# ParBLiSS/kmerind

Measured on AMD Instinct MI355X. Metric: kmers_per_sec_indexed, higher is better.
Workload: dtype u64

## Files before the change

### kmerind_amd/csrc/kmi_superkmer.h

```cpp
#pragma once

namespace kmi {

constexpr int kRecNShift = 38, kRecHashShift = 43;
constexpr uint64_t kSkPadW1 = ~0ull;
constexpr int kRecEdgeShift = 32;
constexpr uint32_t kSkEdgeWindows = 3;
__device__ __forceinline__ uint32_t rec_hash18(uint64_t w1) { return (uint32_t)(w1 >> kRecHashShift) & 0x3ffffu; }
__device__ __forceinline__ uint32_t rec_fine_sub(uint64_t w1) { return (rec_hash18(w1) >> 3) & 127u; }

constexpr int kSkThreads = 512;
constexpr int kSkRoundTiles = 24;
constexpr int kSkListCap = 32;

struct SkRound {
  uint64_t t; uint32_t ei, total; uint32_t eo[kSkRoundTiles + 1]; uint64_t nt; uint32_t nei;
};
__device__ __forceinline__ bool sk_plan(const uint32_t *__restrict__ ent_cnt, uint64_t te, uint64_t t, uint32_t ei, SkRound &r) {
  while (t < te && ei >= ent_cnt[t]) { ++t; ei = 0; }
  if (t >= te) return false;
  r.t = t; r.ei = ei; r.eo[0] = 0;
  r.nt = t + kSkRoundTiles; r.nei = 0;
  bool cut = false;
#pragma unroll
// ... 406 lines not shown
constexpr int kSlackLCap = kSlackLT + (kSlackLineRecs - 1) * kSubPerCoarse;
__global__ __launch_bounds__(kPartThreads) void sk_scatter_fine_slack_lines_kernel(const uint64_t *__restrict__ recs, uint64_t *__restrict__ out,
                                                                                 const uint64_t *__restrict__ wg_off, const uint64_t *__restrict__ coarse_end,
                                                                                 uint32_t groups, const uint64_t *__restrict__ fine_region,
                                                                                 const uint32_t *__restrict__ fine_cap, uint32_t *__restrict__ fine_cnt,
                                                                                 uint32_t *__restrict__ fine_kmers, uint32_t *__restrict__ flags) {
  constexpr int NB = kSubPerCoarse, T = kSlackLT, PT = T / kPartThreads, SCAP = kSlackLCap, L = kSlackLineRecs, MAXG = SCAP / L + NB;
  static_assert(kPartThreads / NB == L && T % kPartThreads == 0, "one carry slot per thread: eight threads per bucket");
  __shared__ ulonglong2 s_stage[SCAP];
  __shared__ uint32_t s_cnt[NB];
  __shared__ uint32_t s_k[NB];
  __shared__ uint32_t s_lofs[NB];
  __shared__ uint32_t s_emit[NB];
  __shared__ uint32_t s_old[NB];
  __shared__ uint32_t s_lbase[NB];
  __shared__ uint64_t s_dst[NB];
  __shared__ uint32_t s_part[NB / kWave];
  __shared__ uint32_t s_ng;
  __shared__ uint8_t s_linebkt[MAXG];
  const uint32_t gpp = groups / kFineParts;
  const uint32_t c = blockIdx.x / kFineParts, h = blockIdx.x % kFineParts;
  const uint64_t b = wg_off[(uint64_t)(h * gpp) * kNumCoarse + c];
  const uint64_t e = (h + 1 < (uint32_t)kFineParts) ? wg_off[(uint64_t)((h + 1) * gpp) * kNumCoarse + c] : coarse_end[c];
  if (b >= e) return;
  const uint64_t region = fine_region[c];
  const uint32_t cap = fine_cap[c];
  if (threadIdx.x < NB) { s_cnt[threadIdx.x] = 0; s_k[threadIdx.x] = 0; }
  const uint32_t cb = threadIdx.x / L, cj = threadIdx.x % L;
  ulonglong2 carry = make_ulonglong2(0, 0);
  uint32_t my_carry = 0;
  lds_barrier();
  const ulonglong2 *src = reinterpret_cast<const ulonglong2 *>(recs);
  ulonglong2 raw[PT];
  auto load_tile = [&](uint64_t t0) {
#pragma unroll
    for (int j = 0; j < PT; ++j) {
      uint64_t i = t0 + (uint64_t)j * kPartThreads + threadIdx.x;
      i = (i < e) ? i : e - 1;
      raw[j] = src[i];
    }
  };
  auto take = [&](uint32_t f, uint32_t n) -> uint64_t {
    const uint32_t at = atomicAdd(&fine_cnt[c * NB + f], n);
    if ((uint64_t)at + n > (uint64_t)cap) { atomicOr(&flags[34], 1u); return ~0ull; }
    return region + (uint64_t)f * cap + at;
  };
  load_tile(b);
  for (uint64_t t0 = b; t0 < e; t0 += T) {
    const uint32_t nt = (uint32_t)((e - t0 < (uint64_t)T) ? (e - t0) : (uint64_t)T);
    ulonglong2 rec[PT];
    uint32_t bk[PT], rk[PT];
#pragma unroll
    for (int j = 0; j < PT; ++j) {
      const uint32_t li = j * kPartThreads + threadIdx.x;
      rec[j] = raw[j];
      bk[j] = 0xffffffffu;
      if (li < nt) {
        bk[j] = rec_fine_sub(rec[j].y);
        rk[j] = atomicAdd(&s_cnt[bk[j]], 1u);
        atomicAdd(&s_k[bk[j]], ((uint32_t)(rec[j].y >> kRecNShift) & 31u) + 1u);
      }
    }
    if (t0 + T < e) load_tile(t0 + T);
    lds_barrier();
    uint32_t cnt = 0, emit = 0, ng = 0, inc = 0;
    if (threadIdx.x < NB) {
      cnt = s_cnt[threadIdx.x];
      const uint32_t km = s_k[threadIdx.x];
      s_k[threadIdx.x] = 0;
      emit = cnt & ~(uint32_t)(L - 1);
      ng = emit / L;
      inc = wave_inclusive_sum_dpp(cnt | (ng << 16));
      if (lane_id() == kWave - 1) s_part[wave_id()] = inc;
      if (km) atomicAdd(&fine_kmers[c * NB + threadIdx.x], km);
      s_dst[threadIdx.x] = emit ? take(threadIdx.x, emit) : ~0ull;
    }
    lds_barrier();
    if (threadIdx.x < NB) {
      const uint32_t pre = wave_id() ? s_part[0] : 0u;
      const uint32_t ex = pre + inc - (cnt | (ng << 16));
      const uint32_t lo = ex & 0xffffu, lb = ex >> 16;
      s_lofs[threadIdx.x] = lo; s_emit[threadIdx.x] = emit; s_old[threadIdx.x] = my_carry; s_lbase[threadIdx.x] = lb;
      for (uint32_t i = 0; i < ng; ++i) s_linebkt[lb + i] = (uint8_t)threadIdx.x;
      if (threadIdx.x == NB - 1) s_ng = lb + ng;
      s_cnt[threadIdx.x] = cnt - emit;
      my_carry = cnt - emit;
    }
    lds_barrier();
    if (cj < s_old[cb]) s_stage[s_lofs[cb] + cj] = carry;
#pragma unroll
    for (int j = 0; j < PT; ++j)
      if (bk[j] != 0xffffffffu) s_stage[s_lofs[bk[j]] + rk[j]] = rec[j];
    lds_barrier();
    {
      const uint32_t n_groups = s_ng, l8 = threadIdx.x & (uint32_t)(L - 1);
      for (uint32_t g = threadIdx.x / L; g < n_groups; g += kPartThreads / L) {
        const uint32_t f = s_linebkt[g];
        const uint64_t d = s_dst[f];
        const uint32_t i = (g - s_lbase[f]) * L + l8;
        if (d != ~0ull) reinterpret_cast<ulonglong2 *>(out)[d + i] = s_stage[s_lofs[f] + i];
      }
      const uint32_t rem = s_cnt[cb], base = s_lofs[cb] + s_emit[cb];
      if (cj < rem) carry = s_stage[base + cj];
    }
    lds_barrier();
  }
  {
    if (threadIdx.x < NB) s_dst[threadIdx.x] = my_carry ? take(threadIdx.x, (uint32_t)L) : ~0ull;
    lds_barrier();
    const uint32_t rem = s_cnt[cb];
    const uint64_t d = s_dst[cb];
    if (rem && d != ~0ull) reinterpret_cast<ulonglong2 *>(out)[d + cj] = cj < rem ? carry : make_ulonglong2(kEmptyKey, kSkPadW1);
  }
}

__global__ __launch_bounds__(1024) void sk_zero_kernel(uint32_t *__restrict__ a, uint32_t na, uint32_t *__restrict__ b, uint32_t nb,
                                                     uint32_t *__restrict__ c, uint32_t nc, uint32_t *__restrict__ flags, uint32_t f0, uint32_t f1,
                                                     uint32_t g0, uint32_t g1) {
  const uint32_t i = blockIdx.x * blockDim.x + threadIdx.x, stride = gridDim.x * blockDim.x;
  for (uint32_t x = i; x < na; x += stride) a[x] = 0;
  for (uint32_t x = i; x < nb; x += stride) b[x] = 0;
  for (uint32_t x = i; x < nc; x += stride) c[x] = 0;
  if (i >= f0 && i < f1) flags[i] = 0;
  if (i >= g0 && i < g1) flags[i] = 0;
}

__global__ __launch_bounds__(kPartThreads) void sk_recv_hist_kernel(const uint64_t *__restrict__ recs, uint64_t n, uint32_t *__restrict__ wg_hist,
                                                                   unsigned long long *__restrict__ n_kmers) {
  __shared__ uint32_t s_h[kNumCoarse];
  __shared__ unsigned long long s_k;
  if (threadIdx.x < kNumCoarse) s_h[threadIdx.x] = 0;
  if (threadIdx.x == 0) s_k = 0ull;
  lds_barrier();
  const uint64_t chunk = part_chunk(n, gridDim.x, PartCfg<2>::TILE);
  const uint64_t b = (uint64_t)blockIdx.x * chunk, e = (b + chunk < n) ? b + chunk : n;
  unsigned long long km = 0;
  for (uint64_t i = b + threadIdx.x; i < e; i += blockDim.x) {
    const uint64_t w1 = recs[2 * i + 1];
    atomicAdd(&s_h[rec_hash18(w1) >> 10], 1u);
    km += ((uint32_t)(w1 >> kRecNShift) & 31u) + 1u;
  }
  km = wave_reduce_sum(km);
  if (lane_id() == 0 && km) atomicAdd(&s_k, km);
  lds_barrier();
  if (threadIdx.x < kNumCoarse) wg_hist[(uint64_t)blockIdx.x * kNumCoarse + threadIdx.x] = s_h[threadIdx.x];
  if (threadIdx.x == 0 && s_k) atomicAdd(n_kmers, s_k);
}

#ifndef KMI_SK_H1
#define KMI_SK_H1 1536
#endif
#ifndef KMI_SK_T1_DUP
#define KMI_SK_T1_DUP 0.5f
#endif
#ifndef KMI_SK_FILL
#define KMI_SK_FILL 80
#endif
#ifndef KMI_SK_NT
#define KMI_SK_NT 1024
#endif
#ifndef KMI_SK_LDS_KB
#define KMI_SK_LDS_KB 160
#endif
#ifndef KMI_SK_HASH24
#define KMI_SK_HASH24 1
#endif
__device__ __forceinline__ uint32_t sk_slot_hash(uint64_t key) {
#if KMI_SK_HASH24
  const uint32_t lo = (uint32_t)key, hi = (uint32_t)(key >> 32);
  uint32_t h = __umul24(lo, 0x9E3779u);
  h += __umul24(__builtin_amdgcn_alignbit(hi, lo, 24), 0x85EBCBu);
  h += __umul24(hi >> 16, 0xC2B2AFu);
#else
  uint32_t h = ((uint32_t)key ^ ((uint32_t)(key >> 32) * 0x85EBCA6Bu)) * 0x9E3779B1u;
#endif
  h ^= h >> 15;
  return h;
}
__device__ __forceinline__ uint32_t sk_slot_of(uint32_t h, uint32_t cap) { return __umul24(h >> 16, cap) >> 16; }

#ifndef KMI_SK_PROBE_ATTR
#define KMI_SK_PROBE_ATTR __forceinline__
#endif
__device__ KMI_SK_PROBE_ATTR uint32_t sk_probe_insert(lds_u64_t *tkeys, lds_u32_t *tvals, lds_u32_t *distinct, lds_u32_t *overflow,
                                                         const lds_u64_t *q, const lds_u32_t *qw, uint32_t first, uint32_t cnt,
                                                         uint32_t cap, uint32_t last, uint32_t limit, uint32_t pending) {
  const uint32_t lane = lane_id();
  bool claimed = false;
  if (lane < cnt) {
    const uint64_t key = q[first + lane];
    const uint32_t wt = qw[first + lane];
    const uint32_t s0 = sk_slot_of(sk_slot_hash(key), cap);
    uint32_t s = s0;
    uint64_t c = __atomic_load_n(&tkeys[s], __ATOMIC_RELAXED);
    for (;;) {
      while (c != key && c != kEmptyKey && s - s0 < 64u) { ++s; c = __atomic_load_n(&tkeys[s], __ATOMIC_RELAXED); }
      if (c == key) break;
      if (c != kEmptyKey || s >= last) { *overflow = 1; s = last; break; }
      uint64_t expected = kEmptyKey;
      if (__atomic_compare_exchange_n(&tkeys[s], &expected, key, false, __ATOMIC_RELAXED, __ATOMIC_RELAXED)) { claimed = true; break; }
      c = expected;
    }
    __atomic_fetch_add(&tvals[s], wt, __ATOMIC_RELAXED);
  }
  const unsigned long long cm = __ballot(claimed);
  const uint32_t add = (uint32_t)__popcll(cm) + pending;
  if (add >= 16u || (add && cnt < 64u)) {
    if (lane == 0 && __atomic_fetch_add(distinct, add, __ATOMIC_RELAXED) + add >= limit) *overflow = 1;
    return 0u;
  }
  return add;
}


#ifndef KMI_SK_OVF
#define KMI_SK_OVF 448
#endif
constexpr int kSkOvf = KMI_SK_OVF;
#ifndef KMI_SK_TICKET_PLAIN
#define KMI_SK_TICKET_PLAIN 1
#endif
#ifndef KMI_SK_EMIT_BLOCK
#define KMI_SK_EMIT_BLOCK 1
#endif
template <int OWN_>
struct SkTab2 {
  static constexpr int NT = KMI_SK_NT, NWAVES = NT / kWave;
  static constexpr int OWN = OWN_;
  static constexpr int H1 = KMI_SK_H1, S1 = H1 + 64, L1 = H1 * 3 / 4;
  static constexpr int FIXED = NWAVES * (OWN + kMissQ * 12) + S1 * 20 + kSkOvf * 16 + 2560;
  static constexpr int S2 = ((KMI_SK_LDS_KB * 1024 - FIXED) / 12) / 64 * 64;
  static constexpr int CAP2 = S2 - 64, LIMIT2 = CAP2 * KMI_SK_FILL / 100;
};

template <bool CANON, int OWN_, bool SPECIAL>
#ifndef KMI_SK_MIN_WAVES
#define KMI_SK_MIN_WAVES 4
#endif
__global__ __launch_bounds__(KMI_SK_NT, KMI_SK_MIN_WAVES) void sk_reduce_kernel(const uint64_t *__restrict__ recs, const uint64_t *__restrict__ rec_off, uint32_t k,
                                                        const uint64_t *__restrict__ kmer_off ,
                                                        uint64_t *__restrict__ tmp_keys, uint32_t *__restrict__ tmp_vals,
                                                        uint32_t *__restrict__ out_cnt, uint32_t *__restrict__ flags,
                                                        uint32_t *__restrict__ queue , uint32_t n_buckets,
                                                        uint32_t start_bits, uint32_t lp, float inv_dup,
                                                        const uint64_t *__restrict__ fine_region = nullptr, const uint32_t *__restrict__ fine_cap = nullptr,
                                                        const uint32_t *__restrict__ fine_cnt = nullptr) {
  auto records_of = [&](uint32_t bb, uint64_t &lo, uint64_t &hi) {
    if (fine_cnt) {
      const uint32_t cap = fine_cap[bb >> 7], cnt = fine_cnt[bb];
      lo = fine_region[bb >> 7] + (uint64_t)(bb & 127u) * cap; hi = lo + (cnt < cap ? cnt : cap);
    }
    else { lo = rec_off[bb]; hi = rec_off[bb + 1]; }
  };
  using T = SkTab2<OWN_>;
  constexpr int NWAVES = T::NWAVES;
  constexpr uint64_t W1_INIT = ~0ull;
  enum { C_DIST = 0, C_OVF = 1, C_SPC = 2, C_SPS = 3, C_EMIT = 4, C_SP = 5, C_OVN = 6, C_T1N = 8, C_LVL = 9, C_NEXT = 10  };
  __shared__ uint64_t s_tk[T::S2];
  __shared__ uint32_t s_tv[T::S2];
  __shared__ ulonglong2 s_r[T::S1];
  __shared__ uint32_t s_rc[T::S1];
  __shared__ ulonglong2 s_ovf[kSkOvf];
  __shared__ uint64_t s_missq[NWAVES * kMissQ];
  __shared__ uint32_t s_missw[NWAVES * kMissQ];
  __shared__ uint8_t s_own[NWAVES * T::OWN];
  __shared__ uint32_t s_ctl[12];
  __shared__ uint32_t s_stack[320];
  const uint32_t lane = lane_id(), wv = wave_id();
  lds_u64_t *const tkeys = (lds_u64_t *)s_tk;
  lds_u32_t *const tvals = (lds_u32_t *)s_tv;
  lds_u32_t *const tdist = (lds_u32_t *)&s_ctl[C_DIST];
  lds_u32_t *const tovf = (lds_u32_t *)&s_ctl[C_OVF];
  uint64_t *const mq = s_missq + wv * kMissQ;
  uint32_t *const mw = s_missw + wv * kMissQ;
  uint8_t *const wown = s_own + wv * T::OWN;
  const uint32_t kb = 2u * k;
  const uint32_t kmask_hi = kb >= 64u ? 0xffffffffu : ((1u << (kb - 32u)) - 1u);
  const uint32_t pad = 64u - kb;
  const bool use_t1_known = inv_dup > 0.f;
  for (uint32_t i = threadIdx.x; i < (uint32_t)(NWAVES * T::OWN / 4); i += T::NT) reinterpret_cast<uint32_t *>(s_own)[i] = 0;
  for (uint32_t i = threadIdx.x; i < (uint32_t)T::S2; i += T::NT) { s_tk[i] = kEmptyKey; s_tv[i] = 0; }
  for (uint32_t i = threadIdx.x; i < (uint32_t)T::S1; i += T::NT) { s_r[i] = make_ulonglong2(kEmptyKey, W1_INIT); s_rc[i] = 0; }
  for (uint32_t i = threadIdx.x; i < (uint32_t)(NWAVES * kMissQ); i += T::NT) s_missq[i] = 0;
  if (threadIdx.x < 12) s_ctl[threadIdx.x] = 0;
  if (threadIdx.x == 0) { s_ctl[C_NEXT] = atomicAdd(queue, 1u); s_ctl[C_NEXT + 1] = atomicAdd(queue, 1u); }
  lds_barrier();
  uint32_t b = __builtin_amdgcn_readfirstlane(s_ctl[C_NEXT]), b1 = __builtin_amdgcn_readfirstlane(s_ctl[C_NEXT + 1]);
  uint32_t par = 0;
  auto share_of = [&](uint32_t n, uint32_t &lo, uint32_t &hi) {
    const uint32_t share = (n + NWAVES - 1) / NWAVES;
    lo = wv * share < n ? wv * share : n;
    hi = lo + share < n ? lo + share : n;
  };
  uint64_t cur_rb = 0, cur_re = 0, cur_k0 = 0, cur_k1 = 0;
  ulonglong2 pf = make_ulonglong2(0, 0);
  if (b < n_buckets) {
    records_of(b, cur_rb, cur_re); cur_k0 = kmer_off[b]; cur_k1 = kmer_off[b + 1];
    uint32_t lo, hi;
    share_of((uint32_t)(cur_re - cur_rb), lo, hi);
    if (lo + lane < hi) pf = reinterpret_cast<const ulonglong2 *>(recs)[cur_rb + lo + lane];
  }
  auto vm_landed = [] { __builtin_amdgcn_s_waitcnt(0x0F70); };
  vm_landed();
  uint32_t mn = 0, pending = 0, my_claims = 0, hbits = 0, hmask = 0, hval = 0;
  auto to_table = [&](uint64_t key, uint32_t kw, bool v) {
    const uint32_t h = sk_slot_hash(key);
    const uint32_t slot = sk_slot_of(h, (uint32_t)T::CAP2);
    v = v && (h & hmask) == hval;
    if (SPECIAL && v && key == kEmptyKey) { s_ctl[C_SPS] = 1; atomicAdd(&s_ctl[C_SPC], kw); v = false; }
    const uint64_t c0 = __atomic_load_n(&s_tk[slot], __ATOMIC_RELAXED), c1 = __atomic_load_n(&s_tk[slot + 1u], __ATOMIC_RELAXED);
    bool hit0 = v && c0 == key;
    const bool hit1 = v && c1 == key;
    bool won = false;
    if (v && c0 == kEmptyKey) {
      const unsigned long long old = atomicCAS((unsigned long long *)&s_tk[slot], (unsigned long long)kEmptyKey, (unsigned long long)key);
      won = old == kEmptyKey;
      hit0 = won || old == key;
    }
    my_claims += won ? 1u : 0u;
    if (hit0 || hit1) atomicAdd(&s_tv[slot + (hit0 ? 0u : 1u)], kw);
    const bool miss = v && !hit0 && !hit1;
    const unsigned long long mm = __ballot(miss);
    if (mm) {
      const uint32_t pos = mn + __builtin_amdgcn_mbcnt_hi((uint32_t)(mm >> 32), __builtin_amdgcn_mbcnt_lo((uint32_t)mm, 0u));
      if (miss) { mq[pos] = key; mw[pos] = kw; }
      mn += (uint32_t)__popcll(mm);
      if (mn >= (uint32_t)kWave) {
        pending = sk_probe_insert(tkeys, tvals, tdist, tovf, (const lds_u64_t *)mq, (const lds_u32_t *)mw, mn - kWave, kWave, (uint32_t)T::CAP2,
                                  (uint32_t)T::S2 - 1u, (uint32_t)T::LIMIT2, pending);
        mn -= kWave;
      }
    }
  };
  uint64_t *const cas_dummy = mq + kWave + lane;
  auto to_table2 = [&](uint64_t ka, bool va, uint64_t kc, bool vc, uint32_t kw) {
    const uint32_t hA = sk_slot_hash(ka), hC = sk_slot_hash(kc);
    const uint32_t sa = sk_slot_of(hA, (uint32_t)T::CAP2), sc = sk_slot_of(hC, (uint32_t)T::CAP2);
    va = va && (hA & hmask) == hval; vc = vc && (hC & hmask) == hval;
    if (SPECIAL) {
      if (va && ka == kEmptyKey) { s_ctl[C_SPS] = 1; atomicAdd(&s_ctl[C_SPC], kw); va = false; }
      if (vc && kc == kEmptyKey) { s_ctl[C_SPS] = 1; atomicAdd(&s_ctl[C_SPC], kw); vc = false; }
    }
    const uint64_t a0 = __atomic_load_n(&s_tk[sa], __ATOMIC_RELAXED), a1 = __atomic_load_n(&s_tk[sa + 1u], __ATOMIC_RELAXED);
    const uint64_t c0 = __atomic_load_n(&s_tk[sc], __ATOMIC_RELAXED), c1 = __atomic_load_n(&s_tk[sc + 1u], __ATOMIC_RELAXED);
    const bool ta = va && a0 == kEmptyKey, tc = vc && c0 == kEmptyKey;
    const unsigned long long oa = atomicCAS((unsigned long long *)(ta ? &s_tk[sa] : cas_dummy), (unsigned long long)kEmptyKey, (unsigned long long)ka);
    const unsigned long long oc = atomicCAS((unsigned long long *)(tc ? &s_tk[sc] : cas_dummy), (unsigned long long)kEmptyKey, (unsigned long long)kc);
    const bool wa_ = ta && oa == kEmptyKey, wc_ = tc && oc == kEmptyKey;
    const bool ha0 = va && (a0 == ka || wa_ || (ta && oa == ka)), hc0 = vc && (c0 == kc || wc_ || (tc && oc == kc));
    const bool ha1 = va && !ha0 && a1 == ka, hc1 = vc && !hc0 && c1 == kc;
    my_claims += (wa_ ? 1u : 0u) + (wc_ ? 1u : 0u);
    atomicAdd(&s_tv[sa + (ha1 ? 1u : 0u)], (ha0 || ha1) ? kw : 0u);
    atomicAdd(&s_tv[sc + (hc1 ? 1u : 0u)], (hc0 || hc1) ? kw : 0u);
    const bool ma = va && !ha0 && !ha1, mc = vc && !hc0 && !hc1;
    const unsigned long long mma = __ballot(ma), mmc = __ballot(mc);
    if (mma | mmc) {
      if (ma) { const uint32_t pos = mn + __builtin_amdgcn_mbcnt_hi((uint32_t)(mma >> 32), __builtin_amdgcn_mbcnt_lo((uint32_t)mma, 0u)); mq[pos] = ka; mw[pos] = kw; }
      mn += (uint32_t)__popcll(mma);
      if (mn >= (uint32_t)kWave) {
        pending = sk_probe_insert(tkeys, tvals, tdist, tovf, (const lds_u64_t *)mq, (const lds_u32_t *)mw, mn - kWave, kWave, (uint32_t)T::CAP2,
                                  (uint32_t)T::S2 - 1u, (uint32_t)T::LIMIT2, pending);
        mn -= kWave;
      }
      if (mc) { const uint32_t pos = mn + __builtin_amdgcn_mbcnt_hi((uint32_t)(mmc >> 32), __builtin_amdgcn_mbcnt_lo((uint32_t)mmc, 0u)); mq[pos] = kc; mw[pos] = kw; }
      mn += (uint32_t)__popcll(mmc);
      if (mn >= (uint32_t)kWave) {
        pending = sk_probe_insert(tkeys, tvals, tdist, tovf, (const lds_u64_t *)mq, (const lds_u32_t *)mw, mn - kWave, kWave, (uint32_t)T::CAP2,
                                  (uint32_t)T::S2 - 1u, (uint32_t)T::LIMIT2, pending);
        mn -= kWave;
      }
    }
  };
  auto expand = [&](uint64_t w0, uint64_t w1, uint32_t wt, uint32_t n) {
    const uint32_t nu = (n + 1u) >> 1;
    const uint32_t inc = wave_inclusive_sum_dpp(nu);
    const uint32_t pre = inc - nu;
    const uint32_t total = __builtin_amdgcn_readlane(inc, kWave - 1);
    if (total == 0u) return;
    if (nu) wown[pre] = (uint8_t)(lane + 1u);
    uint32_t carry = 0;
    const uint32_t top_sh = kb - 34u;
    for (uint32_t g0 = 0; g0 < total; g0 += kWave) {
      const uint32_t g = g0 + lane;
      const bool act = g < total;
      uint32_t o = act ? (uint32_t)wown[g] : 0u;
      o = wave_inclusive_max_dpp(o);
      o = o > carry ? o : carry;
      carry = __builtin_amdgcn_readlane(o, kWave - 1);
      const int rl = (int)((o ? o - 1u : 0u) << 2);
      const uint32_t j = 2u * (g - (uint32_t)__builtin_amdgcn_ds_bpermute(rl, (int)pre));
      const uint32_t a0 = (uint32_t)__builtin_amdgcn_ds_bpermute(rl, (int)(uint32_t)w0), a1 = (uint32_t)__builtin_amdgcn_ds_bpermute(rl, (int)(uint32_t)(w0 >> 32));
      const uint32_t a2 = (uint32_t)__builtin_amdgcn_ds_bpermute(rl, (int)(uint32_t)w1), a3 = (uint32_t)__builtin_amdgcn_ds_bpermute(rl, (int)(uint32_t)(w1 >> 32));
      const uint32_t kw = (uint32_t)__builtin_amdgcn_ds_bpermute(rl, (int)wt);
      const bool two = act && j + 1u <= ((a3 >> (kRecNShift - 32)) & 31u);
      const bool w1sel = j >= 16u;
      const uint32_t bit = (2u * j) & 31u;
      const uint32_t b0 = w1sel ? a1 : a0, b1 = w1sel ? a2 : a1, b2 = w1sel ? a3 : a2;
      const uint32_t rc_lo = __builtin_amdgcn_alignbit(b1, b0, bit);
      const uint32_t rc_hi = __builtin_amdgcn_alignbit(b2, b1, bit) & kmask_hi;
      const uint32_t r_hi = __builtin_bitreverse32(rc_lo), r_lo = __builtin_bitreverse32(rc_hi);
      const uint32_t s_hi = ~(((r_hi >> 1) & 0x55555555u) | ((r_hi << 1) & 0xAAAAAAAAu));
      const uint32_t s_lo = ~(((r_lo >> 1) & 0x55555555u) | ((r_lo << 1) & 0xAAAAAAAAu));
      const uint32_t fw_lo = __builtin_amdgcn_alignbit(s_hi, s_lo, pad), fw_hi = s_hi >> pad;
      const uint32_t rc2_lo = __builtin_amdgcn_alignbit(b1, b0, bit + 2u);
      const uint32_t rc2_hi = __builtin_amdgcn_alignbit(b2, b1, bit + 2u) & kmask_hi;
      const uint32_t fw2_lo = (fw_lo << 2) | (((rc2_hi >> top_sh) & 3u) ^ 3u);
      const uint32_t fw2_hi = __builtin_amdgcn_alignbit(fw_hi, fw_lo, 30u) & kmask_hi;
      const uint64_t rc = (uint64_t)rc_lo | ((uint64_t)rc_hi << 32), fw = (uint64_t)fw_lo | ((uint64_t)fw_hi << 32);
      const uint64_t rc2 = (uint64_t)rc2_lo | ((uint64_t)rc2_hi << 32), fw2 = (uint64_t)fw2_lo | ((uint64_t)fw2_hi << 32);
#ifndef KMI_SK_INSERT1
      to_table2(CANON ? (fw < rc ? fw : rc) : fw, act, CANON ? (fw2 < rc2 ? fw2 : rc2) : fw2, two, kw);
#else
      to_table(CANON ? (fw < rc ? fw : rc) : fw, kw, act);
      to_table(CANON ? (fw2 < rc2 ? fw2 : rc2) : fw2, kw, two);
#endif
    }
    if (nu) wown[pre] = 0;
    const uint32_t batch_claims = __builtin_amdgcn_readlane(wave_inclusive_sum_dpp(my_claims), kWave - 1);
    my_claims = 0;
    pending += batch_claims;
    if (pending >= 32u) {
      if (lane == 0 && atomicAdd(&s_ctl[C_DIST], pending) + pending >= (uint32_t)T::LIMIT2) s_ctl[C_OVF] = 1;
      pending = 0;
    }
  };
#ifdef KMI_SK_TIMING
  unsigned long long acc[8] = {0, 0, 0, 0, 0, 0, 0, 0}, tq = 0;
#define TQ_MARK(i) { const unsigned long long now_ = clock64(); acc[i] += now_ - tq; tq = now_; }
#else
#define TQ_MARK(i)
#endif
  while (b < n_buckets) {
    uint32_t q_next = 0;
    if (threadIdx.x == 0) {
      uint32_t q_at = 0;
#if KMI_SK_TICKET_PLAIN
      asm volatile("" : "+v"(q_at));
#endif
      q_next = atomicAdd(queue + q_at, 1u);
    }
    const uint64_t rb = cur_rb, re = cur_re, tmp0 = cur_k0, tmp1 = cur_k1;
    const uint32_t n_rec = (uint32_t)(re - rb);
    const ulonglong2 *const src = reinterpret_cast<const ulonglong2 *>(recs) + rb;
    uint32_t r_lo, r_hi;
    share_of(n_rec, r_lo, r_hi);
    const ulonglong2 first = pf;
    uint64_t nx_rb = 0, nx_re = 0, nx_k0 = 0, nx_k1 = 0;
    if (b1 < n_buckets) { records_of(b1, nx_rb, nx_re); nx_k0 = kmer_off[b1]; nx_k1 = kmer_off[b1 + 1]; }
    auto prefetch_next = [&]() {
      uint32_t nlo, nhi;
      share_of((uint32_t)(nx_re - nx_rb), nlo, nhi);
      pf = reinterpret_cast<const ulonglong2 *>(recs)[nlo + lane < nhi ? nx_rb + nlo + lane : rb];
    };
    if (threadIdx.x == 0) {
      uint32_t hb = start_bits > 8u ? 8u : start_bits;
      if (use_t1_known && n_rec) {
        const float pred = (float)(tmp1 - tmp0) * inv_dup;
        float room = 0.88f * (float)T::LIMIT2 * (float)(1u << hb);
        while (hb < 8u && pred > room) { ++hb; room *= 2.f; }
      }
      const uint32_t np = n_rec ? (1u << hb) : 0u;
      for (uint32_t v = 0; v < np; ++v) s_stack[v] = hb | (v << 8);
      s_ctl[C_SP] = np; s_ctl[C_EMIT] = 0; s_ctl[C_LVL] = hb;
    }
    bool first_pass = true;
    lds_barrier();
#ifdef KMI_SK_TIMING
    tq = clock64();
#endif
    if (n_rec != 0u) do {
      const uint32_t sp = s_ctl[C_SP];
      const uint32_t pass = s_stack[sp - 1];
      const uint32_t fbits = pass & 0xffu, fval = pass >> 8;
      lds_barrier();
      if (threadIdx.x == 0) s_ctl[C_SP] = sp - 1;
      const bool use_t1 = use_t1_known ? inv_dup <= KMI_SK_T1_DUP : fbits < 2u;
      const uint32_t dead = lp > 2u ? lp - 2u : 0u, rmax = 3u - dead;
      const uint32_t rbits = fbits < rmax ? fbits : rmax, rmask = ((1u << rbits) - 1u) << dead, rval = (fval & ((1u << rbits) - 1u)) << dead;
      hbits = fbits - rbits; hmask = (1u << hbits) - 1u; hval = fval >> rbits;
      mn = 0; pending = 0; my_claims = 0;
      {
        ulonglong2 rec = first;
        if (!first_pass) { rec = make_ulonglong2(0, 0); if (r_lo + lane < r_hi) rec = src[r_lo + lane]; vm_landed(); }
        for (uint32_t r0 = r_lo; r0 < r_hi; r0 += kWave) {
          if (__atomic_load_n(&s_ctl[C_OVF], __ATOMIC_RELAXED)) break;
          const bool have = r0 + lane < r_hi;
          ulonglong2 nxt = rec;
          if (r0 + kWave + lane < r_hi) nxt = src[r0 + kWave + lane];
          uint32_t n = (have && rec.y != kSkPadW1) ? ((uint32_t)(rec.y >> kRecNShift) & 31u) + 1u : 0u;
          if ((rec_hash18(rec.y) & rmask) != rval) n = 0;
          bool direct = n != 0u;
          if (use_t1) {
            if (direct && rec.x != kEmptyKey) {
              uint32_t h = ((uint32_t)rec.x ^ (uint32_t)(rec.x >> 32)) * 0x9E3779B1u ^ ((uint32_t)rec.y ^ (uint32_t)(rec.y >> 32)) * 0x85EBCA6Bu;
              h ^= h >> 15;
              const uint32_t s0 = ((h >> 16) * (uint32_t)T::H1) >> 16;
              for (uint32_t s = s0; direct && s < s0 + 8u; s += 4u) {
                ulonglong2 e[4];
#pragma unroll
                for (int i = 0; i < 4; ++i) e[i] = s_r[s + i];
                int hit = -1, free_ = -1;
#pragma unroll
                for (int i = 3; i >= 0; --i) {
                  const bool same = e[i].x == rec.x && e[i].y == rec.y, empty = e[i].x == kEmptyKey;
                  if (same) { hit = i; free_ = -1; } else if (empty) { free_ = i; hit = -1; }
                }
                if (hit >= 0) { atomicAdd(&s_rc[s + hit], 1u); direct = false; }
                else if (free_ >= 0) {
                  if (__atomic_load_n(&s_ctl[C_T1N], __ATOMIC_RELAXED) >= (uint32_t)T::L1) break;
                  const unsigned long long old = atomicCAS((unsigned long long *)&s_r[s + free_].x, (unsigned long long)kEmptyKey, (unsigned long long)rec.x);
                  if (old == kEmptyKey) {
                    __atomic_store_n(&s_r[s + free_].y, rec.y, __ATOMIC_RELAXED);
                    atomicAdd(&s_rc[s + free_], 1u);
                    atomicAdd(&s_ctl[C_T1N], 1u);
                    direct = false;
                  } else if (old == rec.x && __atomic_load_n(&s_r[s + free_].y, __ATOMIC_RELAXED) == rec.y) {
                    atomicAdd(&s_rc[s + free_], 1u);
                    direct = false;
                  } else break;
                }
              }
            }
            if (direct) {
              const uint32_t oi = atomicAdd(&s_ctl[C_OVN], 1u);
              if (oi < (uint32_t)kSkOvf) { s_ovf[oi] = rec; direct = false; }
            }
          }
          if (__any(direct)) { TQ_MARK(0) expand(rec.x, rec.y, 1u, direct ? n : 0u); TQ_MARK(1) }
          vm_landed();
          rec = nxt;
        }
      }
      TQ_MARK(0)
      if (first_pass && threadIdx.x == 0) s_ctl[C_NEXT + par] = q_next;
      lds_barrier();
      TQ_MARK(2)
      vm_landed();
      if (use_t1) {
        const uint32_t n_ovf = s_ctl[C_OVN] < (uint32_t)kSkOvf ? s_ctl[C_OVN] : (uint32_t)kSkOvf;
        constexpr uint32_t PER1 = ((uint32_t)T::S1 + NWAVES - 1) / NWAVES;
        const uint32_t per_o = (n_ovf + NWAVES - 1) / NWAVES;
        const uint32_t t_lo = wv * PER1, t_hi = t_lo + PER1 < (uint32_t)T::S1 ? t_lo + PER1 : (uint32_t)T::S1;
        const uint32_t o_lo = wv * per_o < n_ovf ? wv * per_o : n_ovf, o_hi = o_lo + per_o < n_ovf ? o_lo + per_o : n_ovf;
        const uint32_t n_mine = (t_hi - t_lo) + (o_hi - o_lo);
        for (uint32_t i0 = 0; i0 < n_mine; i0 += kWave) {
          const uint32_t i = i0 + lane;
          uint64_t w0 = kEmptyKey, w1 = 0; uint32_t wt = 0;
          if (i < t_hi - t_lo) {
            const uint32_t s = t_lo + i;
            const ulonglong2 ent = s_r[s];
            w0 = ent.x; w1 = ent.y; wt = s_rc[s];
            if (w0 != kEmptyKey) { s_r[s] = make_ulonglong2(kEmptyKey, W1_INIT); s_rc[s] = 0; }
          } else if (i < n_mine) {
            const ulonglong2 ent = s_ovf[o_lo + (i - (t_hi - t_lo))];
            w0 = ent.x; w1 = ent.y; wt = 1u;
          }
          uint32_t n = wt ? ((uint32_t)(w1 >> kRecNShift) & 31u) + 1u : 0u;
          if (__atomic_load_n(&s_ctl[C_OVF], __ATOMIC_RELAXED)) n = 0;
          if (__any(n != 0u)) expand(w0, w1, wt, n);
        }
      }
      if (mn) {
        pending = sk_probe_insert(tkeys, tvals, tdist, tovf, (const lds_u64_t *)mq, (const lds_u32_t *)mw, 0u, mn, (uint32_t)T::CAP2, (uint32_t)T::S2 - 1u,
                                  (uint32_t)T::LIMIT2, pending);
        mn = 0;
      }
      if (pending && lane == 0 && atomicAdd(&s_ctl[C_DIST], pending) + pending >= (uint32_t)T::LIMIT2) s_ctl[C_OVF] = 1;
      if (first_pass) prefetch_next();
      first_pass = false;
      TQ_MARK(3)
      lds_barrier();
      TQ_MARK(4)
      const bool lost = s_ctl[C_OVF] != 0u;
      lds_barrier();
      vm_landed();
      if (threadIdx.x == 0) { s_ctl[C_DIST] = 0; s_ctl[C_OVF] = 0; s_ctl[C_T1N] = 0; s_ctl[C_OVN] = 0; }
      if (lost) {
        for (uint32_t i = threadIdx.x; i < (uint32_t)T::S2; i += T::NT) { s_tk[i] = kEmptyKey; s_tv[i] = 0; }
        if (threadIdx.x == 0) {
          s_ctl[C_SPC] = 0; s_ctl[C_SPS] = 0;
          if (fbits >= 18u) atomicOr(&flags[2], 1u);
          else {
            uint32_t best = 0, best_n = 0;
            for (uint32_t l = 0; l <= 8u; ++l) {
              const uint32_t c = __hip_atomic_load(&flags[16 + l], __ATOMIC_RELAXED, __HIP_MEMORY_SCOPE_AGENT);
              if (c > best_n) { best_n = c; best = l; }
            }
            uint32_t target = best > fbits ? best : fbits + 1u;
            if (target > fbits + 6u) target = fbits + 6u;
            uint32_t spn = s_ctl[C_SP];
            for (uint32_t v = 0; v < (1u << (target - fbits)); ++v) s_stack[spn++] = target | ((fval | (v << fbits)) << 8);
            s_ctl[C_SP] = spn;
            if (target > s_ctl[C_LVL]) s_ctl[C_LVL] = target;
          }
        }
        lds_barrier();
        continue;
      }
      {
        uint32_t *s_out = &s_ctl[C_EMIT];
#if KMI_SK_EMIT_BLOCK
        constexpr int EI = (T::S2 + T::NT - 1) / T::NT;
        uint64_t ek[EI]; uint32_t ev[EI], eo[EI];
#pragma unroll
        for (int i = 0; i < EI; ++i) {
          const uint32_t s = threadIdx.x + (uint32_t)i * T::NT;
          ek[i] = kEmptyKey; ev[i] = 0;
          if (i < EI - 1 || s < (uint32_t)T::S2) { ek[i] = s_tk[s]; ev[i] = s_tv[s]; }
        }
        uint32_t total = 0;
#pragma unroll
        for (int i = 0; i < EI; ++i) {
          const unsigned long long m = __ballot(ek[i] != kEmptyKey);
          eo[i] = total + __builtin_amdgcn_mbcnt_hi((uint32_t)(m >> 32), __builtin_amdgcn_mbcnt_lo((uint32_t)m, 0u));
          total += (uint32_t)__popcll(m);
        }
        uint32_t block = 0;
        if (total) {
          if (lane == 0) block = atomicAdd(s_out, total);
          block = __builtin_amdgcn_readfirstlane(block);
        }
        const uint64_t o0 = tmp0 + block;
#pragma unroll
        for (int i = 0; i < EI; ++i) {
          const uint32_t s = threadIdx.x + (uint32_t)i * T::NT;
          if (ek[i] != kEmptyKey) { tmp_keys[o0 + eo[i]] = ek[i]; tmp_vals[o0 + eo[i]] = ev[i]; s_tk[s] = kEmptyKey; s_tv[s] = 0; }
        }
#else
        for (uint32_t s = threadIdx.x; s < (uint32_t)((T::S2 + kWave - 1) / kWave * kWave); s += T::NT) {
          uint64_t key = kEmptyKey; uint32_t val = 0;
          if (s < (uint32_t)T::S2) { key = s_tk[s]; val = s_tv[s]; }
          const bool used = key != kEmptyKey;
          const uint32_t pos = wave_alloc(s_out, used);
          if (used) { tmp_keys[tmp0 + pos] = key; tmp_vals[tmp0 + pos] = val; s_tk[s] = kEmptyKey; s_tv[s] = 0; }
        }
#endif
        lds_barrier();
        if (threadIdx.x == 0) {
          if (s_ctl[C_SPS]) {
            const uint32_t pos = atomicAdd(s_out, 1u);
            tmp_keys[tmp0 + pos] = kEmptyKey;
            tmp_vals[tmp0 + pos] = s_ctl[C_SPC];
          }
          s_ctl[C_SPC] = 0; s_ctl[C_SPS] = 0;
          s_tv[T::S2 - 1] = 0;
        }
      }
      lds_barrier();
      TQ_MARK(5)
    } while (s_ctl[C_SP] != 0u);
    else {
      if (threadIdx.x == 0) s_ctl[C_NEXT + par] = q_next;
      uint32_t nlo, nhi;
      share_of((uint32_t)(nx_re - nx_rb), nlo, nhi);
      if (nlo + lane < nhi) pf = reinterpret_cast<const ulonglong2 *>(recs)[nx_rb + nlo + lane];
      vm_landed();
    }
    if (threadIdx.x == 0) {
      out_cnt[b] = s_ctl[C_EMIT];
      if (n_rec && (s_ctl[C_LVL] || start_bits)) atomicAdd(&flags[16 + (s_ctl[C_LVL] > 8u ? 8u : s_ctl[C_LVL])], 1u);
    }
    lds_barrier();
    const uint32_t b2 = __builtin_amdgcn_readfirstlane(s_ctl[C_NEXT + par]);
    b = b1; b1 = b2; par ^= 1u;
    cur_rb = nx_rb; cur_re = nx_re; cur_k0 = nx_k0; cur_k1 = nx_k1;
    TQ_MARK(6)
  }
#ifdef KMI_SK_TIMING
  if (lane == 0) for (int i = 0; i < 8; ++i) atomicAdd(&reinterpret_cast<unsigned long long *>(flags + 48)[i], acc[i]);
#endif
}

}
```

Baseline: 182.5 billion.

## Make first tier-1 probe branch-free and wave-aggregate counter atomics

Restructures the tier-1 record probe so every lane loads the first four-slot group, then does one predicated CAS and one count atomic instead of running a divergent per-lane loop. The claim counter and the overflow-slot counter are now bumped once per wave via ballot and popcount, with mbcnt giving each lane its offset. This is meant to cut wave divergence and LDS atomic contention. The cost is that every lane now issues atomics, with CAS redirected to a `cas_dummy` location and zero-adds for non-participating lanes. The old bail-out on a contended CAS is also dropped, which slightly changes the probing behaviour.

After: 189.3 billion (median of 6 runs). 3.7% higher.

```diff
diff --git a/kmerind_amd/csrc/kmi_superkmer.h b/kmerind_amd/csrc/kmi_superkmer.h
--- a/kmerind_amd/csrc/kmi_superkmer.h
+++ b/kmerind_amd/csrc/kmi_superkmer.h
@@ -732,6 +732,7 @@
   }
   auto vm_landed = [] { __builtin_amdgcn_s_waitcnt(0x0F70); };
   vm_landed();
+  auto lds_landed = [] { __builtin_amdgcn_s_waitcnt(0xC07F); };
   uint32_t mn = 0, pending = 0, my_claims = 0, hbits = 0, hmask = 0, hval = 0;
   auto to_table = [&](uint64_t key, uint32_t kw, bool v) {
     const uint32_t h = sk_slot_hash(key);
@@ -921,39 +922,68 @@
           if ((rec_hash18(rec.y) & rmask) != rval) n = 0;
           bool direct = n != 0u;
           if (use_t1) {
-            if (direct && rec.x != kEmptyKey) {
-              uint32_t h = ((uint32_t)rec.x ^ (uint32_t)(rec.x >> 32)) * 0x9E3779B1u ^ ((uint32_t)rec.y ^ (uint32_t)(rec.y >> 32)) * 0x85EBCA6Bu;
-              h ^= h >> 15;
-              const uint32_t s0 = ((h >> 16) * (uint32_t)T::H1) >> 16;
-              for (uint32_t s = s0; direct && s < s0 + 8u; s += 4u) {
-                ulonglong2 e[4];
+            uint32_t h = ((uint32_t)rec.x ^ (uint32_t)(rec.x >> 32)) * 0x9E3779B1u ^ ((uint32_t)rec.y ^ (uint32_t)(rec.y >> 32)) * 0x85EBCA6Bu;
+            h ^= h >> 15;
+            const uint32_t s0 = ((h >> 16) * (uint32_t)T::H1) >> 16;
+            ulonglong2 e[4];
+#pragma unroll
+            for (int i = 0; i < 4; ++i) e[i] = s_r[s0 + i];
+            lds_landed();
+            const uint32_t t1n = __atomic_load_n(&s_ctl[C_T1N], __ATOMIC_RELAXED);
+            const bool cand = direct && rec.x != kEmptyKey;
+            uint32_t at = 4u; bool same_at = false;
+#pragma unroll
+            for (int i = 3; i >= 0; --i) {
+              const bool same = e[i].x == rec.x && e[i].y == rec.y, empty = e[i].x == kEmptyKey;
+              at = (same || empty) ? (uint32_t)i : at;
+              same_at = same ? true : (empty ? false : same_at);
+            }
+            const bool full = cand && at == 4u;
+            const bool hit = cand && same_at;
+            const bool may_claim = cand && !same_at && at < 4u && t1n < (uint32_t)T::L1;
+            const uint32_t slot = s0 + (at & 3u);
+            const unsigned long long old = atomicCAS(may_claim ? &s_r[slot].x : (unsigned long long *)cas_dummy, (unsigned long long)kEmptyKey, (unsigned long long)rec.x);
+            const bool won = may_claim && old == kEmptyKey;
+            if (won) __atomic_store_n(&s_r[slot].y, rec.y, __ATOMIC_RELAXED);
+            bool twin = may_claim && old == rec.x;
+            if (__any(twin)) twin = twin && __atomic_load_n(&s_r[slot].y, __ATOMIC_RELAXED) == rec.y;
+            const bool counted = hit || won || twin;
+            atomicAdd(&s_rc[slot], counted ? 1u : 0u);
+            const unsigned long long wm = __ballot(won);
+            if (wm && lane == 0) atomicAdd(&s_ctl[C_T1N], (uint32_t)__popcll(wm));
+            direct = direct && !counted;
+            if (__any(direct)) {
+              if (full) {
+                const uint32_t s = s0 + 4u;
 #pragma unroll
                 for (int i = 0; i < 4; ++i) e[i] = s_r[s + i];
-                int hit = -1, free_ = -1;
+                int hit2 = -1, free_ = -1;
 #pragma unroll
                 for (int i = 3; i >= 0; --i) {
                   const bool same = e[i].x == rec.x && e[i].y == rec.y, empty = e[i].x == kEmptyKey;
-                  if (same) { hit = i; free_ = -1; } else if (empty) { free_ = i; hit = -1; }
+                  if (same) { hit2 = i; free_ = -1; } else if (empty) { free_ = i; hit2 = -1; }
                 }
-                if (hit >= 0) { atomicAdd(&s_rc[s + hit], 1u); direct = false; }
-                else if (free_ >= 0) {
-                  if (__atomic_load_n(&s_ctl[C_T1N], __ATOMIC_RELAXED) >= (uint32_t)T::L1) break;
-                  const unsigned long long old = atomicCAS((unsigned long long *)&s_r[s + free_].x, (unsigned long long)kEmptyKey, (unsigned long long)rec.x);
-                  if (old == kEmptyKey) {
+                if (hit2 >= 0) { atomicAdd(&s_rc[s + hit2], 1u); direct = false; }
+                else if (free_ >= 0 && __atomic_load_n(&s_ctl[C_T1N], __ATOMIC_RELAXED) < (uint32_t)T::L1) {
+                  const unsigned long long old2 = atomicCAS((unsigned long long *)&s_r[s + free_].x, (unsigned long long)kEmptyKey, (unsigned long long)rec.x);
+                  if (old2 == kEmptyKey) {
                     __atomic_store_n(&s_r[s + free_].y, rec.y, __ATOMIC_RELAXED);
                     atomicAdd(&s_rc[s + free_], 1u);
                     atomicAdd(&s_ctl[C_T1N], 1u);
                     direct = false;
-                  } else if (old == rec.x && __atomic_load_n(&s_r[s + free_].y, __ATOMIC_RELAXED) == rec.y) {
+                  } else if (old2 == rec.x && __atomic_load_n(&s_r[s + free_].y, __ATOMIC_RELAXED) == rec.y) {
                     atomicAdd(&s_rc[s + free_], 1u);
                     direct = false;
-                  } else break;
+                  }
                 }
               }
-            }
-            if (direct) {
-              const uint32_t oi = atomicAdd(&s_ctl[C_OVN], 1u);
-              if (oi < (uint32_t)kSkOvf) { s_ovf[oi] = rec; direct = false; }
+              const unsigned long long dm = __ballot(direct);
+              if (dm) {
+                uint32_t base = 0;
+                if (lane == 0) base = atomicAdd(&s_ctl[C_OVN], (uint32_t)__popcll(dm));
+                const uint32_t oi = __builtin_amdgcn_readfirstlane(base) + __builtin_amdgcn_mbcnt_hi((uint32_t)(dm >> 32), __builtin_amdgcn_mbcnt_lo((uint32_t)dm, 0u));
+                if (direct && oi < (uint32_t)kSkOvf) { s_ovf[oi] = rec; direct = false; }
+              }
             }
           }
           if (__any(direct)) { TQ_MARK(0) expand(rec.x, rec.y, 1u, direct ? n : 0u); TQ_MARK(1) }
```
